# mit-acl/roman

Hardware: AMD Instinct MI355X
Metric: submap-pair alignments/sec + p50 latency at n=m=200 objects, d=512 (higher is better)
Workload: dtype f64 (fixed-point SpMV sums); 1 GPU; config 3: batch of 256 submap pairs per GPU, n=200 m=200 d=512, method=semanticgrav (xyz + 512-d descriptors + gravity prior); p50 latency measured on config 2 (single pair); pairs_per_call=256, n=200, m=200, d=512, method=semanticgrav, batches_in_flight=3

## Files before the change

roman_amd/csrc/kernels.hip.h:

```cpp
#pragma once
#include <hip/hip_cooperative_groups.h>
#include <hip/hip_runtime.h>
#include <stdint.h>
#include <type_traits>
#include "../../include/roman_hip.h"

namespace roman {

constexpr int WAVE = 64;
constexpr int STREAM_MAXL = 3072;

struct DevParams {
    roman_params_t p;
    double sig2;
    double sin_unc;
    double x_eps;
    double x_mindist;
    int32_t single;
    int32_t gravity;
    int32_t F;
    int32_t max_compact;
    int32_t gmode;
    int32_t diag_one;
    int32_t keep_all;
// ... 2625 lines not shown
            }
            queued += (uint32_t)__popcll(act);
            while (queued >= 64u * FILL_E) evaluate(64u * FILL_E);
        }
    }
    while (queued > 0u) evaluate(min(queued, 64u * (uint32_t)FILL_E));
    return upper;
}

template <bool GRAV, typename IdxT, bool QUAD>
__global__ void __launch_bounds__(1024) k_fill(DevParams D, const ProbDesc* __restrict__ probs,
                                               ProbState* __restrict__ st,
                                               const BatchTotals* __restrict__ tot,
                                               const ItemDesc* __restrict__ items,
                                               const double* __restrict__ tabPool,
                                               const int32_t* __restrict__ li, const int32_t* __restrict__ lj,
                                               const double* __restrict__ ls,
                                               const double* __restrict__ lza, const double* __restrict__ lzb,
                                               const uint32_t* __restrict__ rowCnt,
                                               const unsigned long long* __restrict__ maskPool,
                                               const uint32_t* __restrict__ prefPool,
                                               const uint32_t* __restrict__ rowPos,
                                               const uint32_t* __restrict__ sliceWidth,
                                               const uint32_t* __restrict__ sliceBase,
                                               IdxT* __restrict__ cols, double* __restrict__ vals, int TC, int RPB ,
                                               const uint32_t* __restrict__ permPool )
{
    extern __shared__ __attribute__((aligned(16))) unsigned char smem[];
    double* cS = reinterpret_cast<double*>(smem);
    double* cZa = cS + TC;
    double* cZb = cZa + (GRAV ? TC : 0);
    int32_t* cI = reinterpret_cast<int32_t*>(cZb + (GRAV ? TC : 0));
    int32_t* cJ = cI + TC;
    uint32_t* cBase = reinterpret_cast<uint32_t*>(cJ + TC);
    uint32_t* cPos = cBase + TC;
    uint32_t* rings = cPos + TC;
    const int tid = threadIdx.x, nt = blockDim.x;
    const int lane = tid & 63, w = tid >> 6, wpb = nt >> 6;
    FillRows R;
    R.s = reinterpret_cast<double*>(rings + (size_t)wpb * 3 * FILL_Q); R.za = R.s + FILL_RPB; R.zb = R.za + FILL_RPB;
    R.k = reinterpret_cast<int32_t*>(R.zb + FILL_RPB); R.i = R.k + FILL_RPB; R.j = R.i + FILL_RPB; R.base = reinterpret_cast<uint32_t*>(R.j + FILL_RPB);
    uint32_t* qK = rings + (size_t)w * 3 * FILL_Q;
    uint32_t* qQ = qK + FILL_Q;
    uint32_t* qE = qQ + FILL_Q;
    const int nItems = tot->items;
    const int gpu_ = max(1, FILL_RPB / RPB);
    const int nUnits = (nItems + gpu_ - 1) / gpu_;
    const int Gx_ = (nUnits + 7) >> 3;
    for (int sIdx_ = blockIdx.x; (sIdx_ >> 3) < Gx_; sIdx_ += gridDim.x) {
        const int u_ = (sIdx_ & 7) * Gx_ + (sIdx_ >> 3);
        if (u_ >= nUnits) continue;
        const int tEnd_ = min(nItems, (u_ + 1) * gpu_);
        for (int t = u_ * gpu_; t < tEnd_; ) {
        ItemDesc it = items[t];
        const int b = it.b;
        int te_ = t + 1;
        while (te_ < tEnd_ && items[te_].b == b) ++te_;
        const int nIt_ = te_ - t;
        t = te_;
        if (uni_i(st[b].kind) == 1) {
        const ProbDesc pd = probs[b];
        const int L = st[b].L;
        const int64_t lo = pd.liveOff, mo = st[b].maskOff, no = st[b].nnzOff;
        const int nrows = min(nIt_ * RPB, L - it.row0);
        const double* TA = tabPool + pd.tabOff;
        const double* TB = TA + (int64_t)pd.n1 * pd.n1;
        const bool ldscol = L <= TC;
        __syncthreads();
        for (int r = tid; r < nrows; r += nt) {
            const uint32_t pos = (uint32_t)(it.row0 + r);
            const int k = (int)permPool[lo + pos];
            R.k[r] = k; R.i[r] = li[lo + k]; R.j[r] = lj[lo + k]; R.s[r] = ls[lo + k];
            if (GRAV) { R.za[r] = lza[lo + k]; R.zb[r] = lzb[lo + k]; }
            R.base[r] = sliceBase[lo + (pos >> 6)] + (pos & 63u);
        }
        if (ldscol) {
            for (int q = tid; q < L; q += nt) {
                cI[q] = li[lo + q]; cJ[q] = lj[lo + q]; cS[q] = ls[lo + q];
                if (GRAV) { cZa[q] = lza[lo + q]; cZb[q] = lzb[lo + q]; }
                const uint32_t pos = rowPos[lo + q];
                cBase[q] = sliceBase[lo + (pos >> 6)] + (pos & 63u); cPos[q] = pos;
            }
        }
        __syncthreads();
        uint32_t upper = 0u;
        if (ldscol)
            upper = fill_item<GRAV, IdxT, 1, QUAD>(D, pd, L, it.row0, nrows, 0, (L + 63) >> 6, w, wpb, lane, cI, cJ, cS, cZa, cZb, cBase, cPos, TA, TB,
                                                maskPool + mo, prefPool + mo, R, qK, qQ, qE, cols + no, vals + no);
        else {
            const int TCw = TC & ~63;
            for (int q0 = 0; q0 < L; q0 += TCw) {
                const int qn = min(TCw, L - q0);
                if (q0 > 0) __syncthreads();
                for (int q = tid; q < qn; q += nt) {
                    const int64_t g_ = lo + q0 + q;
                    cI[q] = li[g_]; cJ[q] = lj[g_]; cS[q] = ls[g_];
                    if (GRAV) { cZa[q] = lza[g_]; cZb[q] = lzb[g_]; }
                    cPos[q] = rowPos[g_];
                }
                __syncthreads();
                upper += fill_item<GRAV, IdxT, 2, QUAD>(D, pd, L, it.row0, nrows, q0, (qn + 63) >> 6, w, wpb, lane, cI, cJ, cS, cZa, cZb, cBase, cPos, TA, TB,
                                                        maskPool + mo, prefPool + mo, R, qK, qQ, qE, cols + no, vals + no);
            }
        }
        for (int r = w; r < nrows; r += wpb) {
            const uint32_t pos = (uint32_t)(it.row0 + r);
            const int k = (int)permPool[lo + pos];
            const uint32_t width = sliceWidth[lo + (pos >> 6)];
            const int64_t sb = no + sliceBase[lo + (pos >> 6)];
            for (uint32_t e = rowCnt[lo + k] + lane; e < width; e += WAVE) {
                cols[col_pos<QUAD>(sb, pos & 63u, e)] = fb_inert<IdxT>(pos);
                vals[val_pos<QUAD>(sb, pos & 63u, e)] = 0.0;
            }
        }
        if (QUAD && it.row0 + nrows == L && (L & 63)) {
            const uint32_t sl = (uint32_t)(L >> 6);
            const uint32_t width = sliceWidth[lo + sl];
            const int64_t sb = no + sliceBase[lo + sl];
            const uint32_t nfree = 64u - (uint32_t)(L & 63);
            for (uint32_t x = tid; x < nfree * width; x += nt) {
                const uint32_t slot = (uint32_t)(L & 63) + x / width, e = x % width;
                cols[col_pos<QUAD>(sb, slot, e)] = fb_inert<IdxT>(0u);
                vals[val_pos<QUAD>(sb, slot, e)] = 0.0;
            }
        }
        for (int off = 32; off > 0; off >>= 1) upper += __shfl_xor(upper, off);
        if (lane == 0 && upper) atomicAdd(&st[b].nnzUpper, (unsigned long long)upper);
        }
        }
    }
}

constexpr int FILLS_MAXSPI = STREAM_MAXL / 64;

template <bool GRAV, bool FAST>
__device__ __forceinline__ double fill_value(const DevParams& D, double a, double bb, double dza, double dzb, double ss, double sk, double sq)
{
    double c;
    if (GRAV && D.gmode != 3) {
        const double ch = fabs(a - bb);
        const double hm = a > bb ? a : bb;
        double cv = fabs(dza - dzb) - D.sin_unc * hm;
        if (cv < 0.0) cv = 0.0;
        c = sqrt(ch * ch + cv * cv);
    } else {
        c = fabs(a - bb);
    }
    const double sa = fx_exp(((-0.5 * c) * c) / D.sig2);
    if (FAST) return (sa == 0.0) ? 0.0 : fx_cbrt(sa * ss);
    return fuse_pair(D, sa, sk, sq);
}

constexpr uint32_t FILL_ROTATE = 5;

template <bool GRAV, bool FAST, bool OBJ>
__global__ void __launch_bounds__(1024) k_fill_list(DevParams D, int B, const ProbDesc* __restrict__ probs,
                                                    ProbState* __restrict__ st, const BatchTotals* __restrict__ tot,
                                                    const double* __restrict__ tabPool, const double* __restrict__ feats, int NO ,
                                                    const int32_t* __restrict__ li, const int32_t* __restrict__ lj,
                                                    const double* __restrict__ ls,
                                                    const double* __restrict__ lza, const double* __restrict__ lzb,
                                                    const uint16_t* __restrict__ listPool, const uint32_t* __restrict__ listOff,
                                                    const uint32_t* __restrict__ rowCnt,
                                                    const uint32_t* __restrict__ perm, const uint32_t* __restrict__ rowPos,
                                                    const uint32_t* __restrict__ sliceWidth,
                                                    const uint32_t* __restrict__ sliceBase,
                                                    uint16_t* __restrict__ cols, double* __restrict__ vals, int TC, int NG, int SPI )
{
    extern __shared__ __attribute__((aligned(16))) unsigned char smem[];
    double* cS = reinterpret_cast<double*>(smem);
    dbl2_t* sO = reinterpret_cast<dbl2_t*>(cS + TC);
    double* cZa = OBJ ? cS + TC + 8 * NO : cS + TC;
    double* cZb = cZa + ((GRAV && !OBJ) ? TC : 0);
    int32_t* cI = reinterpret_cast<int32_t*>(cZb + ((GRAV && !OBJ) ? TC : 0));
    int32_t* cJ = cI + TC;
    uint32_t* gK = reinterpret_cast<uint32_t*>(cJ + TC);
    uint32_t* gCnt = gK + SPI * 64;
    uint32_t* gOff = gCnt + SPI * 64;
    uint32_t* gQ = gOff + SPI * 64;
    uint32_t* gSB = gQ + SPI + 1;
    uint16_t* cP = reinterpret_cast<uint16_t*>(gSB + SPI + 1);
    const int tid = threadIdx.x, nt = blockDim.x;
    const int lane = tid & 63, w = tid >> 6, nw = nt >> 6;
    const int nGroups = tot->sliceGroups;
    const int Gx = (nGroups + 7) >> 3;
    for (int sIdx = blockIdx.x; (sIdx >> 3) < Gx; sIdx += gridDim.x) {
        const int t = (sIdx & 7) * Gx + (sIdx >> 3);
        if (t < nGroups) {
        int b = 0;
        {
            int lo_ = 0, hi_ = B - 1;
            while (lo_ < hi_) { const int mid = (lo_ + hi_ + 1) >> 1; if (st[mid].sgBase <= t) lo_ = mid; else hi_ = mid - 1; }
            b = lo_;
        }
        const ProbDesc pd = probs[b];
        const int L = st[b].L;
        const int W = (L + 63) >> 6;
        const int64_t lo = pd.liveOff, no = st[b].nnzOff;
        const uint16_t* lists = listPool + st[b].listOff;
        const int ngb = min(NG, W), spib = (W + ngb - 1) / max(ngb, 1);
        const int s_begin = (t - st[b].sgBase) * spib, s_end = min(W, s_begin + spib), ns = max(s_end - s_begin, 0);
        const double* TA = tabPool + pd.tabOff;
        const double* TB = TA + (int64_t)pd.n1 * pd.n1;
        __syncthreads();
        for (int q = tid; q < L; q += nt) {
            cI[q] = li[lo + q]; cJ[q] = lj[lo + q]; cS[q] = ls[lo + q]; cP[q] = (uint16_t)rowPos[lo + q];
            if (GRAV && !OBJ) { cZa[q] = lza[lo + q]; cZb[q] = lzb[lo + q]; }
        }
        if (OBJ) {
            const int pdim = D.p.point_dim;
            for (int o = tid; o < pd.n1 + pd.n2; o += nt) {
                const double* f = feats + (o < pd.n1 ? pd.off1 + o : pd.off2 + (o - pd.n1)) * D.F;
                const int slot = o < pd.n1 ? o : NO + (o - pd.n1);
                sO[2 * slot] = dbl2_t{f[0], pdim > 1 ? f[1] : 0.0};
                sO[2 * slot + 1] = dbl2_t{pdim > 2 ? f[2] : 0.0, 0.0};
            }
        }
        const bool horiz = D.gmode == 1 || D.gmode == 2;
        for (int x = tid; x < ns * 64; x += nt) {
            const int p = s_begin * 64 + x;
            const bool row = p < L;
            gK[x] = row ? perm[lo + p] : 0xffffffffu; gCnt[x] = row ? rowCnt[lo + p] : 0u; gOff[x] = row ? listOff[lo + p] : 0u;
        }
        if (w == 0) {
            const uint32_t wq = (lane < ns) ? (sliceWidth[lo + s_begin + lane] >> 2) : 0u;
            const uint32_t ex = wave_excl_scan(wq, lane);
            if (lane < ns) { gQ[lane] = ex; gSB[lane] = sliceBase[lo + s_begin + lane]; }
            if (lane == ns) gQ[ns] = ex;
        }
        __syncthreads();
        const uint32_t Q = gQ[ns];
        uint32_t upper = 0;
        int si = 0;
        for (uint32_t u = (uint32_t)w; u < Q; u += (uint32_t)nw) {
            while (u >= gQ[si + 1]) ++si;
            const uint32_t g = u - gQ[si];
            const int64_t sb = no + gSB[si];
            const int x = si * 64 + lane;
            const uint32_t kraw = gK[x], cnt = gCnt[x];
            const uint32_t nq = (cnt + 3u) >> 2;
            uint32_t e0 = g << 2;
            if (g < nq) e0 = ((g + (uint32_t)x * FILL_ROTATE) % nq) << 2;
            uint2 qq = make_uint2(0u, 0u);
            if (e0 < cnt) qq = *reinterpret_cast<const uint2*>(lists + gOff[x] + e0);
            const int k = (kraw == 0xffffffffu) ? 0 : (int)kraw;
            const double sk = cS[k];
            const double* TAr = TA + (int64_t)cI[k] * pd.n1;
            const double* TBr = TB + (int64_t)cJ[k] * pd.n2;
            const double zak = (GRAV && !OBJ) ? cZa[k] : 0.0, zbk = (GRAV && !OBJ) ? cZb[k] : 0.0;
            dbl2_t oa0 = {0.0, 0.0}, oa1 = {0.0, 0.0}, ob0 = {0.0, 0.0}, ob1 = {0.0, 0.0};
            if (OBJ) { oa0 = sO[2 * cI[k]]; oa1 = sO[2 * cI[k] + 1]; ob0 = sO[2 * (NO + cJ[k])]; ob1 = sO[2 * (NO + cJ[k]) + 1]; }
            const uint32_t inert = ((uint32_t)L + (uint32_t)lane) | 0x8000u;
            uint32_t cw[4]; double vv[4];
#pragma unroll
            for (int j = 0; j < 4; ++j) {
                const bool have = e0 + (uint32_t)j < cnt;
                const uint32_t qr = ((j < 2 ? qq.x : qq.y) >> (16 * (j & 1))) & 0xffffu;
                const int q = have ? (int)qr : k;
                double a, bb, dza, dzb;
                if (OBJ) {
                    const dbl2_t pa0 = sO[2 * cI[q]], pa1 = sO[2 * cI[q] + 1], pb0 = sO[2 * (NO + cJ[q])], pb1 = sO[2 * (NO + cJ[q]) + 1];
                    const double dxa = oa0.x - pa0.x, dya = oa0.y - pa0.y, dxb = ob0.x - pb0.x, dyb = ob0.y - pb0.y;
                    dza = oa1.x - pa1.x; dzb = ob1.x - pb1.x;
                    const double h2a = dxa * dxa + dya * dya, h2b = dxb * dxb + dyb * dyb;
                    a = horiz ? sqrt(h2a) : sqrt(h2a + dza * dza);
                    bb = horiz ? sqrt(h2b) : sqrt(h2b + dzb * dzb);
                } else {
                    a = TAr[cI[q]]; bb = TBr[cJ[q]];
                    dza = GRAV ? zak - cZa[q] : 0.0; dzb = GRAV ? zbk - cZb[q] : 0.0;
                }
                if (!have) { a = 0.0; bb = 0.0; }
                const double sq = cS[q];
                const double v = fill_value<GRAV, FAST>(D, a, bb, GRAV ? dza : 0.0, GRAV ? dzb : 0.0, sk * sq, sk, sq);
                const bool keep = have && v > D.p.affinityeps;
                cw[j] = keep ? (uint32_t)cP[q] : inert;
                vv[j] = keep ? v : 0.0;
                upper += keep ? 1u : 0u;
            }
            *reinterpret_cast<uint2*>(cols + sb + (int64_t)g * 256 + lane * 4) = make_uint2(cw[0] | (cw[1] << 16), cw[2] | (cw[3] << 16));
            *reinterpret_cast<double2*>(vals + sb + (int64_t)(2 * g) * 128 + lane * 2) = make_double2(vv[0], vv[1]);
            *reinterpret_cast<double2*>(vals + sb + (int64_t)(2 * g + 1) * 128 + lane * 2) = make_double2(vv[2], vv[3]);
        }
        for (int off = 32; off > 0; off >>= 1) upper += __shfl_xor(upper, off);
        if (lane == 0 && upper) atomicAdd(&st[b].nnzUpper, (unsigned long long)upper);
        }
    }
}

__device__ __forceinline__ void dense_entry(const double* __restrict__ M, const double* __restrict__ C, int n, int k, int q, double& mv, double& cv)
{
    const int a = min(k, q), b = max(k, q);
    mv = M[(int64_t)a * n + b]; cv = C[(int64_t)a * n + b];
}

__global__ void __launch_bounds__(256) k_dense_mask(int n, const double* __restrict__ M, const double* __restrict__ C,
                                                    unsigned long long* __restrict__ mask ,
                                                    int* __restrict__ flags )
{
    const int lane = threadIdx.x & 63;
    const int W = (n + 63) >> 6;
    const int nwaves = (int)(gridDim.x * (blockDim.x >> 6));
    for (int k = (int)(blockIdx.x * (blockDim.x >> 6) + (threadIdx.x >> 6)); k < n; k += nwaves) {
        bool cz = false;
        for (int w = 0; w < W; ++w) {
            const int q = (w << 6) + lane;
            bool cand = false;
            if (q < n && q != k) {
                double mv, cv;
                dense_entry(M, C, n, k, q, mv, cv);
                cand = (mv != 0.0) || (cv != 0.0);
                cz = cz || (cand && cv == 0.0);
            }
            const unsigned long long m = __ballot(cand);
            if (lane == 0) mask[(int64_t)k * W + w] = m;
        }
        if (__ballot(cz) != 0ull && lane == 0) atomicOr(flags, 1);
    }
}

__global__ void __launch_bounds__(256) k_dense_range(int n, const double* __restrict__ M, int* __restrict__ flags)
{
    const int lane = threadIdx.x & 63;
    const int nwaves = (int)(gridDim.x * (blockDim.x >> 6));
    bool bad = false;
    for (int k = (int)(blockIdx.x * (blockDim.x >> 6) + (threadIdx.x >> 6)); k < n; k += nwaves)
        for (int q = k + 1 + lane; q < n; q += 64) {
            const double v = M[(int64_t)k * n + q];
            bad = bad || !(v >= 0.0 && v <= 1.0);
        }
    if (__ballot(bad) != 0ull && lane == 0) atomicOr(flags + 1, 1);
}

template <int KIND>
__global__ void __launch_bounds__(256) k_dense_fill(int n, const double* __restrict__ M, const double* __restrict__ C,
                                                    ProbState* __restrict__ st,
                                                    const uint32_t* __restrict__ rowCnt, const uint32_t* __restrict__ rowPos, const uint32_t* __restrict__ perm,
                                                    const uint32_t* __restrict__ sliceWidth, const uint32_t* __restrict__ sliceBase,
                                                    const uint16_t* __restrict__ listPool, const uint32_t* __restrict__ listOff,
                                                    const unsigned long long* __restrict__ mask, const uint32_t* __restrict__ pref,
                                                    uint16_t* __restrict__ cols16, uint32_t* __restrict__ cols32, double* __restrict__ vals)
{
    const uint32_t total = st[0].nnzCap;
    const int64_t no = st[0].nnzOff;
    const int nsl = (n + 63) >> 6, W = nsl;
    const uint16_t* lists = listPool + st[0].listOff;
    unsigned upper = 0;
    for (uint32_t t = blockIdx.x * blockDim.x + threadIdx.x; t < total; t += gridDim.x * blockDim.x) {
        int sl = 0;
        {
            int lo_ = 0, hi_ = nsl - 1;
            while (lo_ < hi_) { const int mid = (lo_ + hi_ + 1) >> 1; if (sliceBase[mid] <= t) lo_ = mid; else hi_ = mid - 1; }
            sl = lo_;
        }
        const uint32_t sb = sliceBase[sl], off = t - sb;
        const uint32_t slot = (off & 255u) >> 2, e = ((off >> 8) << 2) | (off & 3u);
        const int pos = sl * 64 + (int)slot;
        const int k = pos < n ? (int)perm[pos] : -1;
        double val = 0.0;
        if (KIND == 0) {
            uint32_t label = ((uint32_t)n + slot) | 0x8000u;
            if (k >= 0 && e < rowCnt[pos]) {
                const int q = (int)lists[listOff[pos] + e];
                double mv, cv;
                dense_entry(M, C, n, k, q, mv, cv);
                label = rowPos[q] | (cv == 0.0 ? 0x8000u : 0u); val = mv; ++upper;
            }
            cols16[no + t] = (uint16_t)label;
        } else {
            uint32_t label = (uint32_t)(k >= 0 ? pos : 0) | 0x80000000u;
            if (k >= 0 && e < rowCnt[k]) {
                const unsigned long long* mrow = mask + (int64_t)k * W;
                const uint32_t* prow = pref + (int64_t)k * W;
                int lo_ = 0, hi_ = W - 1;
                while (lo_ < hi_) { const int mid = (lo_ + hi_ + 1) >> 1; if (prow[mid] <= e) lo_ = mid; else hi_ = mid - 1; }
                unsigned long long m = mrow[lo_];
                for (uint32_t i = prow[lo_]; i < e; ++i) m &= m - 1ull;
                const int q = (lo_ << 6) + __builtin_ctzll(m);
                double mv, cv;
                dense_entry(M, C, n, k, q, mv, cv);
                label = rowPos[q] | (cv == 0.0 ? 0x80000000u : 0u); val = mv;
                if (q > k) ++upper;
            }
            cols32[no + t] = label;
        }
        vals[no + val_pos<true>(sb, slot, e)] = val;
    }
    for (int off = 32; off > 0; off >>= 1) upper += __shfl_xor(upper, off);
    if ((threadIdx.x & 63) == 0 && upper) atomicAdd(&st[0].nnzUpper, (unsigned long long)upper);
}


struct SolveOut {
    int32_t* assoc_out; int32_t* n_assoc_out; double* T_out; int32_t* status_out;
    roman_stats_t* stats_out; int32_t kmax;
    int32_t* nodesOrig;
    int32_t* nSel;
    double*  uOut;
    unsigned long long* dbg;
};

__device__ __forceinline__ void block_sum2(double& a, double& b, double* red, int& par, int tid, int nw)
{
    for (int off = 32; off > 0; off >>= 1) { a += __shfl_xor(a, off); b += __shfl_xor(b, off); }
    double* rr = red + 32 * par;
    par ^= 1;
    if ((tid & 63) == 0) { rr[2 * (tid >> 6)] = a; rr[2 * (tid >> 6) + 1] = b; }
    __syncthreads();
    double ra = 0.0, rb = 0.0;
    for (int i = 0; i < nw; ++i) { ra += rr[2 * i]; rb += rr[2 * i + 1]; }
    a = ra; b = rb;
}

typedef unsigned int uint4_t __attribute__((ext_vector_type(4)));
template <typename IdxT, int G>
__device__ __forceinline__ void spmv_sell(const double* u, int L, const uint32_t* __restrict__ perm,
                                          const uint32_t* __restrict__ sliceWidth, const uint32_t* __restrict__ sliceBase,
                                          const IdxT* __restrict__ cols, const double* __restrict__ vals,
                                          double* Mu, double* Cu, int tid, int nt)
{
    static_assert(sizeof(IdxT) == 4, "fallback layout: 32-bit column words");
    const int lane = tid & 63, w = tid >> 6, nw = nt >> 6;
    const int nsl = (L + 63) >> 6;
    for (int s = w; s < nsl; s += nw) {
        const int pos = (s << 6) + lane;
        const bool valid = pos < L;
        const uint32_t nq = sliceWidth[s] >> 2;
        const uint4_t* cp = reinterpret_cast<const uint4_t*>(cols + sliceBase[s]) + lane;
        const dbl2_t* vp = reinterpret_cast<const dbl2_t*>(vals + sliceBase[s]) + lane;
        double am = 0.0, ac = 0.0;
        for (uint32_t g0 = 0; g0 < nq; g0 += G) {
            uint4_t c_[G]; dbl2_t v0_[G], v1_[G];
#pragma unroll
            for (int t = 0; t < G; ++t) {
                const uint32_t g = min(g0 + (uint32_t)t, nq - 1u);
// ... 3927 lines not shown
```

roman_amd/csrc/roman_hip.hip:

```cpp
#include <hip/hip_runtime.h>
#include <algorithm>
#include <cmath>
#include <cstdarg>
#include <cstdint>
#include <cstdio>
#include <cstdlib>
#include <cstring>
#include <new>
#include <string>
#include <vector>

#include "kernels.hip.h"

using namespace roman;

namespace {

thread_local std::string g_last_error;

struct DevBuf {
    void* p = nullptr; size_t cap = 0;
    hipError_t ensure(size_t bytes) {
        if (bytes <= cap) return hipSuccess;
        if (p) { hipError_t e = hipFree(p); p = nullptr; cap = 0; if (e != hipSuccess) return e; }
// ... 589 lines not shown
    const int Lneed = (expL + 255) & ~255;
    const int NRc = ((size_t)16 * 2 * ldsPerRow * sizeof(double) + (size_t)std::min(Lneed, 2048) * colBytesC <= c->lds_max) ? 2 : 1;
    int wpb = 16;
    while (wpb > 1 && (size_t)wpb * NRc * ldsPerRow * sizeof(double) + 256 * colBytesC > c->lds_max) wpb >>= 1;
    if ((size_t)wpb * NRc * ldsPerRow * sizeof(double) + 256 * colBytesC > c->lds_max)
        return fail(c, ROMAN_E_TOO_LARGE, "maps of %d objects exceed the LDS table staging of this build", maxN);
    const int ldsPerWave = NRc * ldsPerRow;
    const size_t tabLds = (size_t)wpb * ldsPerWave * sizeof(double);
    int TCc = (int)std::min<size_t>((c->lds_max - tabLds) / colBytesC, 32768) & ~255;
    TCc = std::min(TCc, Lneed);
    const size_t pairLds = tabLds + (size_t)TCc * colBytesC;
    const int pairGrid = c->num_cu * std::max(1, std::min(2048 / (wpb * 64), (int)(c->lds_max / pairLds)));
    int preNR = 0, preWpb = 0, preTC = 0; size_t preLds = 0;
    const int preRow = (2 * std::max(maxN, 1) + 1 + 3) & ~3;
    {
        const char* preEnv = getenv("ROMAN_COUNT_PRE");
        const bool want = (preEnv ? preEnv[0] != '0' : true) && D.pre_invw > 0.0 && std::isfinite(D.pre_invw) && Lneed <= (preEnv ? 16000 : 4096) && maxN <= 32767;
        if (want) {
            const int tc = Lneed;
            for (int wp = PRE_WAVES; wp >= 8; wp -= 4) {
                const size_t need = (size_t)(tc + PRE_COLPAD + 4) * 4 + (size_t)wp * (size_t)count_pre_wave_bytes(preRow, tc);
                if (need <= c->lds_max) { preNR = PRE_NR; preWpb = wp; preTC = tc; preLds = need; break; }
            }
        }
    }

    StageTimer t1(c, ROMAN_STAGE_COUNT_PASS);
    {
        static const char* fusedEnv = getenv("ROMAN_SMALL_FUSED");
        const bool want = smallOut != nullptr && !(fusedEnv && fusedEnv[0] == '0') && D.p.maxiniters >= 1 && D.p.maxlsiters >= 1 && maxTab > 0 &&
                          (c->hist.valid ? c->hist.smallSeen : maxA <= 16 * SMALL_MAXL);
        if (want) {
            SolveOut O;
            int rc = make_solve_out(c, B, sumA, *smallOut, &O);
            if (rc) return rc;
            HIPCHK(c, hipMemsetAsync(WS.queue.as<int>() + 8, 0, sizeof(int), WS.stream));
            const bool fast = D.single && (D.p.single_mode == ROMAN_SINGLE_BOTH || D.p.single_mode == ROMAN_SINGLE_OFFDIAG) && D.p.distance_weight == 1.0 &&
                              D.p.fusion_method != ROMAN_FUSE_ARITHMETIC_MEAN && D.p.fusion_method != ROMAN_FUSE_PRODUCT;
            constexpr size_t ldsSmall = small_lds_bytes();
            const int grid = std::max(1, std::min(B, c->num_cu * 12));
            auto ks = fast ? k_small<true> : k_small<false>;
            hipLaunchKernelGGL(ks, dim3(grid), dim3(64), ldsSmall, WS.stream, D, B, dP, dS, in.feats, in.assoc, WS.tabPool.as<double>(),
                               LP.lp, LP.li, LP.lj, LP.ls, LP.ld, LP.lza, LP.lzb, WS.plp.as<int32_t>(), WS.pld.as<double>(), WS.rowPos.as<uint32_t>(),
                               smallU0, O, WS.queue.as<int>() + 8);
    DBG(c, "k_small");
            static const char* onlyEnv = getenv("ROMAN_SMALL_ONLY");
            D.small_only = (c->hist.valid && !c->hist.generalSeen && !(onlyEnv && onlyEnv[0] == '0')) ? 1 : 0;
            Dout->small_only = D.small_only;
        }
    }
    hipLaunchKernelGGL(k_rowbase, dim3(1), dim3(B > 256 ? 1024 : 256), 0, WS.stream, B, RPB, SZ.capMaskWords, dS, dT, D.small_only, cosScreen ? (const int32_t*)WS.cosDense.as<int32_t>() : (const int32_t*)nullptr);
    DBG(c, "k_rowbase");
    if (!D.small_only) {
    hipLaunchKernelGGL(k_items, dim3(B), dim3(256), 0, WS.stream, RPB, dS, WS.items.as<ItemDesc>());
    DBG(c, "k_items");
    }
    if (sumA > 0 && !D.small_only) {
        const bool needTiled = D.allow_fallback || TCc < Lneed;
        int degGiven = 0;
        for (int tiled = 0; tiled < (needTiled ? 2 : 1); ++tiled) {
            const void* kc = nullptr;
#define ROMAN_KC(GM_) kc = tiled ? (NRc == 2 ? reinterpret_cast<const void*>(k_count<GM_, 2, true>) : reinterpret_cast<const void*>(k_count<GM_, 1, true>)) \
                                 : (NRc == 2 ? reinterpret_cast<const void*>(k_count<GM_, 2, false>) : reinterpret_cast<const void*>(k_count<GM_, 1, false>))
            switch (D.gmode) { case 1: ROMAN_KC(1); break; case 2: ROMAN_KC(2); break; case 3: ROMAN_KC(3); break; default: ROMAN_KC(0); break; }
#undef ROMAN_KC
            const bool usePre = !tiled && preNR > 0;
            if (usePre) {
#define ROMAN_KP(GM_) kc = reinterpret_cast<const void*>(k_count<GM_, 1, false, true>)
                switch (D.gmode) { case 1: ROMAN_KP(1); break; case 2: ROMAN_KP(2); break; case 3: ROMAN_KP(3); break; default: ROMAN_KP(0); break; }
#undef ROMAN_KP
            }
            const size_t ldsK = usePre ? preLds : pairLds;
            const int wpbK = usePre ? preWpb : wpb;
            const int gridK = usePre ? c->num_cu * std::max(1, std::min(2048 / (wpbK * 64), (int)(c->lds_max / ldsK))) : pairGrid;
            const char* wholeEnv = getenv("ROMAN_COUNT_WHOLE");
            const bool wholeP = usePre && (wholeEnv ? wholeEnv[0] != '0' : B >= c->num_cu) && preLds + (size_t)preTC * 4 <= c->lds_max;
            if (wholeP) degGiven = 1;
            HIPCHK(c, dyn_lds(c, kc, ldsK + (wholeP ? (size_t)preTC * 4 : 0)));
            DevParams a_D = D; const ProbDesc* a_dP = dP; const ProbState* a_dS = dS; const BatchTotals* a_dT = dT; const ItemDesc* a_items = WS.items.as<ItemDesc>();
            const double* a_tab = WS.tabPool.as<double>(); const int32_t* a_li = LP.li; const int32_t* a_lj = LP.lj; const double* a_za = LP.lza; const double* a_zb = LP.lzb;
            uint32_t* a_rc = WS.rowCnt.as<uint32_t>(); unsigned long long* a_mask = WS.maskPool.as<unsigned long long>(); uint32_t* a_pref = WS.prefPool.as<uint32_t>();
            int a_TC = usePre ? preTC : TCc, a_lpw = usePre ? preRow : ldsPerWave;
            int a_RPB = wholeP ? -B : RPB;
            const uint16_t* a_qtab = WS.qtabPool.as<uint16_t>();
            void* args[] = {&a_D, &a_dP, &a_dS, &a_dT, &a_items, &a_tab, &a_li, &a_lj, &a_za, &a_zb, &a_rc, &a_mask, &a_pref, &a_TC, &a_lpw, &a_RPB, &a_qtab};
            HIPCHK(c, hipLaunchKernel(kc, dim3(gridK), dim3(wpbK * 64), args, ldsK + (wholeP ? (size_t)preTC * 4 : 0), WS.stream));
        }
    DBG(c, "k_count");
        const char* listsEnv = getenv("ROMAN_LISTS");
        const int fusedLists = listsEnv ? (listsEnv[0] == '0' ? 0 : 1) : (B >= std::max(8, c->num_cu / 8) ? 1 : 0);
        if (fusedLists) {
            static size_t listsStatic = 0;
            if (listsStatic == 0) {
                hipFuncAttributes fa;
                HIPCHK(c, hipFuncGetAttributes(&fa, reinterpret_cast<const void*>(k_lists)));
                listsStatic = std::max<size_t>(fa.sharedSizeBytes, 1);
            }
            const char* llEnv = getenv("ROMAN_LISTS_LDS");
            const size_t room = c->lds_max > listsStatic ? c->lds_max - listsStatic : 0;
            const size_t winBytes = std::min(room, llEnv ? (size_t)std::max(0, atoi(llEnv)) : room) & ~(size_t)15;
            if (winBytes) HIPCHK(c, dyn_lds(c, reinterpret_cast<const void*>(k_lists), winBytes));
            hipLaunchKernelGGL(k_lists, dim3((unsigned)std::max(1, std::min(B, 2 * c->num_cu))), dim3(LISTS_NT), winBytes, WS.stream, B, dP, dS, dT,
                               WS.maskPool.as<unsigned long long>(), WS.listPool.as<uint16_t>(), WS.listOff.as<uint32_t>(),
                               WS.rowCnt.as<uint32_t>(), WS.perm.as<uint32_t>(), WS.rowPos.as<uint32_t>(), LP, PP, (long long)SZ.capList, sort_eq_max(), degGiven,
                               (int)(winBytes / sizeof(uint16_t)));
    DBG(c, "k_lists");
        }
        if (!fusedLists || D.allow_fallback) {
        {
            const int Wexp = (expL + 63) / 64;
            const int tasks = ((Wexp + 7) / 8) * ((std::max(Wexp - 1, 1) + 7) / 8);
            const int T = std::max(tasks, 1);
            hipLaunchKernelGGL(k_mirror, dim3((unsigned)(T * ((B + 7) / 8) * 8)), dim3(512), 0, WS.stream, B, T, dS, WS.maskPool.as<unsigned long long>(), fusedLists);
    DBG(c, "k_mirror");
        }
        hipLaunchKernelGGL(k_rowprefix, dim3(c->num_cu * 2), dim3(1024), 0, WS.stream, dP, dS, dT, WS.items.as<ItemDesc>(),
                           WS.maskPool.as<unsigned long long>(), WS.prefPool.as<uint32_t>(), WS.rowCnt.as<uint32_t>(), RPB, fusedLists);
    DBG(c, "k_rowprefix");
        int sortThr = 1024;
        if (!D.allow_fallback) { int N2 = 64; while (N2 < expL) N2 <<= 1; sortThr = std::max(64, std::min(1024, N2 / 2)); }
        hipLaunchKernelGGL(k_rowsort, dim3(B), dim3(sortThr), 0, WS.stream, dP, dS, dT, WS.rowCnt.as<uint32_t>(), WS.rowPos.as<uint32_t>(), WS.perm.as<uint32_t>(),
                           WS.sliceWidth.as<uint32_t>(), WS.sliceBase.as<uint32_t>(), WS.listOff.as<uint32_t>(), SZ.capList, fusedLists, sort_eq_max());
    DBG(c, "k_rowsort");
        if (!fusedLists) {
        const int upThr = expL <= 256 ? 256 : 1024;
        hipLaunchKernelGGL(k_upper, dim3(c->num_cu * 2 * (1024 / upThr)), dim3(upThr), 0, WS.stream, dP, dS, dT, WS.items.as<ItemDesc>(),
                           WS.maskPool.as<unsigned long long>(), WS.listPool.as<uint16_t>(), WS.listOff.as<uint32_t>(),
                           WS.rowCnt.as<uint32_t>(), WS.perm.as<uint32_t>(), WS.rowPos.as<uint32_t>(), LP, PP, RPB);
    DBG(c, "k_upper");
        }
        }
        hipLaunchKernelGGL(k_slicegeom, dim3(B), dim3(64), 0, WS.stream, dP, dS, WS.rowCnt.as<uint32_t>(), WS.sliceWidth.as<uint32_t>(), WS.sliceBase.as<uint32_t>());
    DBG(c, "k_slicegeom");
    }
    int NG = (int)std::max<int64_t>(1, std::min<int64_t>(FILLS_MAXSPI, (3 * (int64_t)c->num_cu + B / 2) / std::max(B, 1)));
    {
        const int stride = std::max(1, (c->num_cu & ~7) / 8);
        auto gcd = [](int a, int b) { while (b) { const int t = a % b; a = b; b = t; } return a; };
        while (NG > 1 && gcd(stride % NG, NG) != 1) --NG;
    }
    const int Wmax = std::max(1, D.stream_maxL / 64);
    const int SPI = (Wmax + std::min(NG, Wmax) - 1) / std::min(NG, Wmax);
    if (!D.small_only) {
    hipLaunchKernelGGL(k_probscan, dim3(1), dim3(B > 256 ? 1024 : 256), 0, WS.stream, B, NG, SZ.capNnz, dS, dT);
    DBG(c, "k_probscan");
    }
    t1.stop();

    StageTimer t2(c, ROMAN_STAGE_FILL);
    if (sumA > 0 && !D.small_only) {
        const int colBytesF = D.gravity ? 32 : 16;
        const int TCs = D.stream_maxL;
        const int NO = (std::max(maxN, 1) + 1) & ~1;
        const size_t groupLds = sizeof(uint32_t) * (size_t)(3 * SPI * 64 + 2 * (SPI + 1) + 2);
        const bool obj = (size_t)TCs * (16 + 2) + (size_t)64 * NO + groupLds <= c->lds_max;
        const size_t sliceLds = obj ? (size_t)TCs * (16 + 2) + (size_t)64 * NO + groupLds : (size_t)TCs * (colBytesF + 2) + groupLds;
        if (sliceLds > c->lds_max) return fail(c, ROMAN_E_TOO_LARGE, "internal: stream column tile does not fit the LDS");
        const bool fast = D.single && (D.p.single_mode == ROMAN_SINGLE_BOTH || D.p.single_mode == ROMAN_SINGLE_OFFDIAG) && D.p.distance_weight == 1.0 &&
                          D.p.fusion_method != ROMAN_FUSE_ARITHMETIC_MEAN && D.p.fusion_method != ROMAN_FUSE_PRODUCT;
        auto kf = D.gravity ? (fast ? k_fill_list<true, true, false> : k_fill_list<true, false, false>) : (fast ? k_fill_list<false, true, false> : k_fill_list<false, false, false>);
        if (obj) kf = D.gravity ? (fast ? k_fill_list<true, true, true> : k_fill_list<true, false, true>) : (fast ? k_fill_list<false, true, true> : k_fill_list<false, false, true>);
        HIPCHK(c, dyn_lds(c, reinterpret_cast<const void*>(kf), sliceLds));
        const int fillThr = expL <= 256 ? 256 : 1024;
        const int fillWgs = std::max(1, std::min(1024 / fillThr, (int)(c->lds_max / sliceLds)));
        hipLaunchKernelGGL(kf, dim3((unsigned)((c->num_cu & ~7) * fillWgs)), dim3(fillThr), sliceLds, WS.stream,
                           D, B, dP, dS, dT, WS.tabPool.as<double>(), in.feats, NO, LP.li, LP.lj, LP.ls, LP.lza, LP.lzb,
                           WS.listPool.as<uint16_t>(), WS.listOff.as<uint32_t>(), WS.rowCnt.as<uint32_t>(), WS.perm.as<uint32_t>(), WS.rowPos.as<uint32_t>(),
                           WS.sliceWidth.as<uint32_t>(), WS.sliceBase.as<uint32_t>(), WS.cols16.as<uint16_t>(), WS.vals.as<double>(), TCs, NG, SPI);
    DBG(c, "k_fill_list");
        if (D.allow_fallback && (SZ.maxA > D.stream_maxL || D.p.maxiniters < 1 || D.p.maxlsiters < 1)) {
            const int colBytesG = D.gravity ? 40 : 24;
            const size_t ringLds = (size_t)16 * 3 * FILL_Q * sizeof(uint32_t) + (size_t)FILL_RPB * FILL_ROWBYTES;
            static_assert(FILL_RPB >= 128, "the work items of a batch are blocks of at most 128 rows");
            int TCf = (int)std::min<size_t>((c->lds_max - ringLds) / colBytesG, 32768) & ~63;
            TCf = std::min(TCf, std::max(64, (Lneed + 63) & ~63));
            const size_t fillLds = ringLds + (size_t)TCf * colBytesG;
            const int fillGrid = c->num_cu * std::max(1, std::min(2, (int)(c->lds_max / fillLds)));
            if (D.idx16) {
                auto kg = D.gravity ? k_fill<true, uint16_t, true> : k_fill<false, uint16_t, true>;
                HIPCHK(c, dyn_lds(c, reinterpret_cast<const void*>(kg), fillLds));
                hipLaunchKernelGGL(kg, dim3(fillGrid), dim3(1024), fillLds, WS.stream, D, dP, dS, dT, WS.items.as<ItemDesc>(), WS.tabPool.as<double>(),
                                   LP.li, LP.lj, LP.ls, LP.lza, LP.lzb,
                                   WS.rowCnt.as<uint32_t>(), WS.maskPool.as<unsigned long long>(), WS.prefPool.as<uint32_t>(), WS.rowPos.as<uint32_t>(),
                                   WS.sliceWidth.as<uint32_t>(), WS.sliceBase.as<uint32_t>(), WS.cols16.as<uint16_t>(), WS.vals.as<double>(), TCf, RPB, (const uint32_t*)WS.perm.as<uint32_t>());
            } else {
                auto kg = D.gravity ? k_fill<true, uint32_t, true> : k_fill<false, uint32_t, true>;
                HIPCHK(c, dyn_lds(c, reinterpret_cast<const void*>(kg), fillLds));
                hipLaunchKernelGGL(kg, dim3(fillGrid), dim3(1024), fillLds, WS.stream, D, dP, dS, dT, WS.items.as<ItemDesc>(), WS.tabPool.as<double>(),
                                   LP.li, LP.lj, LP.ls, LP.lza, LP.lzb,
                                   WS.rowCnt.as<uint32_t>(), WS.maskPool.as<unsigned long long>(), WS.prefPool.as<uint32_t>(), WS.rowPos.as<uint32_t>(),
                                   WS.sliceWidth.as<uint32_t>(), WS.sliceBase.as<uint32_t>(), WS.cols32.as<uint32_t>(), WS.vals.as<double>(), TCf, RPB, (const uint32_t*)WS.perm.as<uint32_t>());
            }
    DBG(c, "k_fill");
        }
    }
    t2.stop();
    HIPCHK(c, hipMemcpyAsync(WS.pinnedTotals, dT, sizeof(BatchTotals), hipMemcpyDeviceToHost, WS.stream));
    HIPCHK(c, hipEventRecord(WS.totEvent, WS.stream));
    WS.totPending = true; WS.totMaskBound = SZ.maskBound; WS.totSumA = SZ.sumA; WS.totMaxA = SZ.maxA; WS.totEpoch = c->histEpoch;
    HIPCHK(c, hipGetLastError());
    return ROMAN_OK;
}

int enqueue_solve(roman_ctx* c, const DevParams& D, int B, int64_t sumA, int64_t maxA , const double* feats, const int32_t* assoc,
                  const double* u0, bool hascz, int mayFallback , const BatchOut& out)
{
    const size_t R1 = (size_t)std::max<int64_t>(sumA, 1);
    SolveOut O;
    { int rc_ = make_solve_out(c, B, sumA, out, &O); if (rc_) return rc_; }
#ifdef ROMAN_SOLVE_TIMING
    HIPCHK(c, WS.hAux3.ensure(sizeof(unsigned long long) * 16 * (size_t)B));
    HIPCHK(c, hipMemsetAsync(WS.hAux3.p, 0, sizeof(unsigned long long) * 16 * (size_t)B, WS.stream));
    O.dbg = WS.hAux3.as<unsigned long long>();
#endif
    constexpr int NW = SOLVE_WAVES;
    const int Lc = STREAM_MAXL + 64;
    const size_t ldsUp = (size_t)3 * 8 * Lc + sizeof(double) * red_doubles(NW) + sizeof(uint32_t) * (ST_MAXSL + 2) + sizeof(int) * 8 + 16;
    const int wgPerCu = std::max(1, std::min((int)(c->lds_max / ldsUp), 2048 / (NW * 64)));
    const int gridUp = std::max(1, std::min(B, c->num_cu * wgPerCu));

    StageTimer t3(c, ROMAN_STAGE_SOLVE);
    const bool coopPlanned = mayFallback && D.wide != 0 && c->coop_ok;
    if (coopPlanned) {
        HIPCHK(c, WS.wideBar.ensure(sizeof(unsigned) * WIDE_BAR_WORDS));
        HIPCHK(c, WS.fbList.ensure(sizeof(int32_t) * (size_t)B));
        HIPCHK(c, hipMemsetAsync(WS.wideBar.p, 0, sizeof(unsigned) * WIDE_BAR_WORDS, WS.stream));
    }
    hipLaunchKernelGGL(k_skipped, dim3((unsigned)((B + 255) / 256)), dim3(256), 0, WS.stream, B, WS.probs.as<ProbDesc>(), WS.state.as<ProbState>(), O, WS.queue.as<int>(),
                       coopPlanned ? WS.fbList.as<int32_t>() : (int32_t*)nullptr, coopPlanned ? WS.wideBar.as<unsigned>() : (unsigned*)nullptr);
    DBG(c, "k_skipped");
    if (D.small_only) { t3.stop(); HIPCHK(c, hipGetLastError()); return ROMAN_OK; }
    static const char* smallEnv = getenv("ROMAN_SMALL");
    const bool small = !(smallEnv && smallEnv[0] == '0') && D.p.maxiniters >= 1 && D.p.maxlsiters >= 1 &&
                       (c->hist.valid ? c->hist.smallSeen : maxA <= 16 * SMALL_MAXL);
    const int Lc1 = SMALL_MAXL + 64;
    const size_t ldsUp1 = (size_t)3 * 8 * Lc1 + sizeof(double) * red_doubles(1) + sizeof(uint32_t) * (ST_MAXSL + 2) + sizeof(int) * 8 + 16 + (size_t)COO_CAP * 12;
    const int gridUp1 = std::max(1, std::min(B, c->num_cu * 24));
#define ROMAN_LAUNCH_UP(CZ_)                                                                                                  \
    do {                                                                                                                      \
        auto kup = k_solve_up<NW, CZ_, STREAM_MAXL>;                                                                          \
        HIPCHK(c, dyn_lds(c, reinterpret_cast<const void*>(kup), ldsUp)); \
        hipLaunchKernelGGL(kup, dim3(gridUp), dim3(NW * 64), ldsUp, WS.stream, D, B, WS.probs.as<ProbDesc>(), WS.state.as<ProbState>(), feats, assoc, \
                           WS.plp.as<int32_t>(), WS.lp.as<int32_t>(), WS.rowPos.as<uint32_t>(), WS.pld.as<double>(), WS.sliceBase.as<uint32_t>(), \
                           WS.cols16.as<uint16_t>(), WS.vals.as<double>(), u0, O, WS.queue.as<int>(), Lc, small ? SMALL_MAXL + 1 : 0, STREAM_MAXL, (small && c->hist.valid && !c->hist.largeSeen) ? 64 : 1); \
        if (small) {                                                                                                          \
            HIPCHK(c, dyn_lds(c, reinterpret_cast<const void*>(k_solve_up<1, CZ_, SMALL_MAXL>), ldsUp1));                       \
            hipLaunchKernelGGL((k_solve_up<1, CZ_, SMALL_MAXL>), dim3(gridUp1), dim3(64), ldsUp1, WS.stream, D, B, WS.probs.as<ProbDesc>(), WS.state.as<ProbState>(), feats, assoc, \
                               WS.plp.as<int32_t>(), WS.lp.as<int32_t>(), WS.rowPos.as<uint32_t>(), WS.pld.as<double>(), WS.sliceBase.as<uint32_t>(), \
                               WS.cols16.as<uint16_t>(), WS.vals.as<double>(), u0, O, WS.queue.as<int>() + 1, Lc1, 0, SMALL_MAXL, 1); \
        }                                                                                                                     \
    } while (0)
    if (hascz) ROMAN_LAUNCH_UP(true); else ROMAN_LAUNCH_UP(false);
#undef ROMAN_LAUNCH_UP
    DBG(c, "k_solve_up");
    if (mayFallback) {
        HIPCHK(c, WS.vMu.ensure(sizeof(double) * R1)); HIPCHK(c, WS.vCu.ensure(sizeof(double) * R1));
        HIPCHK(c, WS.vMun.ensure(sizeof(double) * R1)); HIPCHK(c, WS.vCun.ensure(sizeof(double) * R1));
        HIPCHK(c, WS.gU.ensure(sizeof(double) * R1)); HIPCHK(c, WS.gUn.ensure(sizeof(double) * R1));
        bool coop = D.wide != 0 && c->coop_ok;
        if (coop) {
            const int G = c->num_cu;
            int a_teams = 0;
            const int perXcd = std::max(1, (G + c->num_xcc - 1) / c->num_xcc);
            {
                constexpr int margin = 2;
                auto cap = [&](int sub) { return (int64_t)WIDE_KW * std::max(1, perXcd / sub - margin) * WIDE_NW * 64; };
                if (mayFallback >= 2 && maxA <= cap(1)) {
                    a_teams = 1;
                    for (int s_ = 2; s_ <= 4; ++s_) if (mayFallback > 6 * s_ && maxA <= cap(s_)) a_teams = s_;
                    if (a_teams == 2 && mayFallback > 18 && G == c->num_cu && maxA <= (int64_t)WIDE_KW * (perXcd / 3) * WIDE_NW * 64) a_teams = 3;
                }
                const char* teamEnv = getenv("ROMAN_WIDE_TEAMS");
                const int forced = teamEnv ? atoi(teamEnv) : c->wide_teams;
                if (teamEnv || c->wide_teams >= 0) a_teams = (forced >= 1 && forced <= 4 && mayFallback >= 1 && maxA <= cap(forced)) ? forced : 0;
            }
            if (a_teams) c->teams_launched = true;
            const int nTeams = a_teams ? 8 * a_teams : 1;
            const int NWGt = a_teams ? std::min(G, 2 * ((perXcd + a_teams - 1) / a_teams) + 8) * WIDE_NW : G * WIDE_NW;
            int a_ucfg = (D.idx16 && a_teams > 0 && maxA >= 8000) ? 1 : 0;
            { const char* e_ = getenv("ROMAN_WIDE_UPPER"); if (e_ && e_[0]) a_ucfg = (D.idx16 && e_[0] != '0') ? 1 : 0; }
            long long a_partStride = (long long)(((size_t)NWGt * WIDE_MAXCH + (size_t)(a_ucfg ? WIDE_MAXBLK : 1) * ((size_t)(maxA + 63) / 64) + 4) * 64 * 2);
            HIPCHK(c, WS.widePart.ensure(sizeof(double) * (size_t)a_partStride * (size_t)nTeams));
            HIPCHK(c, WS.wideSlots.ensure(sizeof(double) * 2 * (size_t)G * WIDE_NRED * (size_t)nTeams));
            DevParams Dv = D; int Bv = B;
            const ProbDesc* a_probs = WS.probs.as<ProbDesc>(); ProbState* a_state = WS.state.as<ProbState>();
            const double* a_feats = feats; const int32_t* a_assoc = assoc;
            const int32_t* a_lp = WS.lp.as<int32_t>(); const double* a_ld = WS.ld.as<double>();
            const uint32_t* a_perm = WS.perm.as<uint32_t>(); const uint32_t* a_rpos = WS.rowPos.as<uint32_t>(); const uint32_t* a_sb = WS.sliceBase.as<uint32_t>();
            const void* a_cols = D.idx16 ? (const void*)WS.cols16.as<uint16_t>() : (const void*)WS.cols32.as<uint32_t>(); const double* a_vals = WS.vals.as<double>();
            double* a_vU = WS.gU.as<double>(); double* a_vX = WS.gUn.as<double>(); double* a_vX2 = WS.vCun.as<double>();
            double* a_s0 = WS.vMu.as<double>(); double* a_s1 = WS.vCu.as<double>(); double* a_s2 = WS.vMun.as<double>();
            int32_t* a_plp = WS.plp.as<int32_t>();
            const double* a_u0 = u0; SolveOut a_O = O;
            double* a_part = WS.widePart.as<double>(); double* a_slots = WS.wideSlots.as<double>(); unsigned* a_bar = WS.wideBar.as<unsigned>();
            int a_bmw = (int)((maxA + 63) / 64) + 1;
            HIPCHK(c, WS.wideBm.ensure(sizeof(unsigned long long) * 3 * (size_t)a_bmw * (size_t)nTeams));
            unsigned long long* a_bm = WS.wideBm.as<unsigned long long>();
            const int64_t wideFixed = (int64_t)wide_fixed_lds(a_bmw);
            int a_xcap = (int)(((int64_t)c->lds_max - 4096 - wideFixed) / (int64_t)sizeof(double)) & ~63;
            if (a_xcap < 0) a_xcap = 0;
            const size_t wideLds = sizeof(double) * (size_t)a_xcap + (size_t)wideFixed;
            int a_ccfg = 6 | (128 << 8) | (4 << 16);
            { const char* e_ = getenv("ROMAN_WIDE_COMPACT"); if (e_ && e_[0]) a_ccfg = (int)strtol(e_, nullptr, 0); }
            int a_ySlots = NWGt / WIDE_NW;
            int a_ycap = a_ucfg ? ((a_xcap / 3) & ~63) : 0;
            if (a_ucfg && a_ycap < 64) a_ucfg = 0;
            if (a_ucfg) {
// ... 2670 lines not shown
```

Before: 180,200 alignments/s.

## Compact live fill work across slices so waves process only non-padding list quads

The sliced fill kernel used to give each wave one quad-group of a 64-row slice, so lanes whose row had no list entries at that depth sat idle or wrote padding. It now processes windows of 256 quad-groups: a ballot marks live lanes, padding entries are written directly, a prefix scan over live counts builds a compacted index, and every lane then takes one live (row, group) pair found by binary search and nth-set-bit. This is meant to cut lane divergence and wasted ALU work on skewed row lengths. The cost is extra barriers per window, more LDS, scattered rather than coalesced stores, and search overhead.

```diff
diff --git a/roman_amd/csrc/kernels.hip.h b/roman_amd/csrc/kernels.hip.h
--- a/roman_amd/csrc/kernels.hip.h
+++ b/roman_amd/csrc/kernels.hip.h
@@ -2801,6 +2801,20 @@
 }
 
 constexpr uint32_t FILL_ROTATE = 5;
+constexpr int FILL_WIN = 256;
+
+__device__ __forceinline__ uint32_t nth_set_bit(uint32_t lo, uint32_t hi, uint32_t n)
+{
+    uint32_t base = 0, v = lo;
+    const uint32_t c = (uint32_t)__popc(lo);
+    if (n >= c) { n -= c; v = hi; base = 32; }
+#pragma unroll
+    for (int s = 16; s > 0; s >>= 1) {
+        const uint32_t cl = (uint32_t)__popc(v & ((1u << s) - 1u));
+        if (n >= cl) { n -= cl; v >>= s; base += (uint32_t)s; }
+    }
+    return base;
+}
 
 template <bool GRAV, bool FAST, bool OBJ>
 __global__ void __launch_bounds__(1024) k_fill_list(DevParams D, int B, const ProbDesc* __restrict__ probs,
@@ -2828,7 +2842,11 @@
     uint32_t* gOff = gCnt + SPI * 64;
     uint32_t* gQ = gOff + SPI * 64;
     uint32_t* gSB = gQ + SPI + 1;
-    uint16_t* cP = reinterpret_cast<uint16_t*>(gSB + SPI + 1);
+    uint32_t* wLo = gSB + SPI + 1;
+    uint32_t* wHi = wLo + FILL_WIN;
+    uint32_t* wSl = wHi + FILL_WIN;
+    uint32_t* wPre = wSl + FILL_WIN;
+    uint16_t* cP = reinterpret_cast<uint16_t*>(wPre + FILL_WIN + 1);
     const int tid = threadIdx.x, nt = blockDim.x;
     const int lane = tid & 63, w = tid >> 6, nw = nt >> 6;
     const int nGroups = tot->sliceGroups;
@@ -2880,26 +2898,62 @@
         __syncthreads();
         const uint32_t Q = gQ[ns];
         uint32_t upper = 0;
-        int si = 0;
-        for (uint32_t u = (uint32_t)w; u < Q; u += (uint32_t)nw) {
-            while (u >= gQ[si + 1]) ++si;
-            const uint32_t g = u - gQ[si];
+        int si1 = 0;
+        for (uint32_t u0 = 0; u0 < Q; u0 += (uint32_t)FILL_WIN) {
+            const uint32_t Wn = min((uint32_t)FILL_WIN, Q - u0);
+            if (u0) __syncthreads();
+            for (uint32_t ul = (uint32_t)w; ul < Wn; ul += (uint32_t)nw) {
+                const uint32_t u = u0 + ul;
+                while (u >= gQ[si1 + 1]) ++si1;
+                const uint32_t g = u - gQ[si1];
+                const bool live = g < ((gCnt[si1 * 64 + lane] + 3u) >> 2);
+                const unsigned long long m = __ballot(live);
+                if (lane == 0) { wLo[ul] = (uint32_t)m; wHi[ul] = (uint32_t)(m >> 32); wSl[ul] = (uint32_t)si1; wPre[ul] = (uint32_t)__popcll(m); }
+                if (!live) {
+                    const int64_t sb = no + gSB[si1];
+                    const uint32_t inert = ((uint32_t)L + (uint32_t)lane) | 0x8000u, i2 = inert | (inert << 16);
+                    *reinterpret_cast<uint2*>(cols + sb + (int64_t)g * 256 + lane * 4) = make_uint2(i2, i2);
+                    *reinterpret_cast<double2*>(vals + sb + (int64_t)(2 * g) * 128 + lane * 2) = make_double2(0.0, 0.0);
+                    *reinterpret_cast<double2*>(vals + sb + (int64_t)(2 * g + 1) * 128 + lane * 2) = make_double2(0.0, 0.0);
+                }
+            }
+            for (uint32_t ul = Wn + (uint32_t)tid; ul < (uint32_t)FILL_WIN; ul += (uint32_t)nt) wPre[ul] = 0u;
+            __syncthreads();
+            if (w == 0) {
+                static_assert(FILL_WIN == 4 * WAVE, "one wave scans the window, four slot quads per lane");
+                uint32_t c[4], s = 0;
+#pragma unroll
+                for (int j = 0; j < 4; ++j) { c[j] = wPre[4 * lane + j]; s += c[j]; }
+                uint32_t ex = wave_excl_scan(s, lane);
+#pragma unroll
+                for (int j = 0; j < 4; ++j) { wPre[4 * lane + j] = ex; ex += c[j]; }
+                if (lane == WAVE - 1) wPre[FILL_WIN] = ex;
+            }
+            __syncthreads();
+            const uint32_t F = wPre[FILL_WIN];
+            for (uint32_t f0 = (uint32_t)uni_i(w) * 64u; f0 < F; f0 += (uint32_t)nt) {
+            uint32_t ul = 0;
+            { uint32_t lo_ = 0, hi_ = Wn - 1u; while (lo_ < hi_) { const uint32_t mid = (lo_ + hi_ + 1u) >> 1; if (wPre[mid] <= f0) lo_ = mid; else hi_ = mid - 1u; } ul = lo_; }
+            const uint32_t f = f0 + (uint32_t)lane;
+            if (f < F) {
+            while (wPre[ul + 1] <= f) ++ul;
+            const int r = (int)nth_set_bit(wLo[ul], wHi[ul], f - wPre[ul]);
+            const int si = (int)wSl[ul];
+            const uint32_t g = u0 + ul - gQ[si];
             const int64_t sb = no + gSB[si];
-            const int x = si * 64 + lane;
+            const int x = si * 64 + r;
             const uint32_t kraw = gK[x], cnt = gCnt[x];
             const uint32_t nq = (cnt + 3u) >> 2;
-            uint32_t e0 = g << 2;
-            if (g < nq) e0 = ((g + (uint32_t)x * FILL_ROTATE) % nq) << 2;
-            uint2 qq = make_uint2(0u, 0u);
-            if (e0 < cnt) qq = *reinterpret_cast<const uint2*>(lists + gOff[x] + e0);
-            const int k = (kraw == 0xffffffffu) ? 0 : (int)kraw;
+            const uint32_t e0 = ((g + (uint32_t)x * FILL_ROTATE) % nq) << 2;
+            const uint2 qq = *reinterpret_cast<const uint2*>(lists + gOff[x] + e0);
+            const int k = (int)kraw;
             const double sk = cS[k];
             const double* TAr = TA + (int64_t)cI[k] * pd.n1;
             const double* TBr = TB + (int64_t)cJ[k] * pd.n2;
             const double zak = (GRAV && !OBJ) ? cZa[k] : 0.0, zbk = (GRAV && !OBJ) ? cZb[k] : 0.0;
             dbl2_t oa0 = {0.0, 0.0}, oa1 = {0.0, 0.0}, ob0 = {0.0, 0.0}, ob1 = {0.0, 0.0};
             if (OBJ) { oa0 = sO[2 * cI[k]]; oa1 = sO[2 * cI[k] + 1]; ob0 = sO[2 * (NO + cJ[k])]; ob1 = sO[2 * (NO + cJ[k]) + 1]; }
-            const uint32_t inert = ((uint32_t)L + (uint32_t)lane) | 0x8000u;
+            const uint32_t inert = ((uint32_t)L + (uint32_t)r) | 0x8000u;
             uint32_t cw[4]; double vv[4];
 #pragma unroll
             for (int j = 0; j < 4; ++j) {
@@ -2926,9 +2980,11 @@
                 vv[j] = keep ? v : 0.0;
                 upper += keep ? 1u : 0u;
             }
-            *reinterpret_cast<uint2*>(cols + sb + (int64_t)g * 256 + lane * 4) = make_uint2(cw[0] | (cw[1] << 16), cw[2] | (cw[3] << 16));
-            *reinterpret_cast<double2*>(vals + sb + (int64_t)(2 * g) * 128 + lane * 2) = make_double2(vv[0], vv[1]);
-            *reinterpret_cast<double2*>(vals + sb + (int64_t)(2 * g + 1) * 128 + lane * 2) = make_double2(vv[2], vv[3]);
+            *reinterpret_cast<uint2*>(cols + sb + (int64_t)g * 256 + r * 4) = make_uint2(cw[0] | (cw[1] << 16), cw[2] | (cw[3] << 16));
+            *reinterpret_cast<double2*>(vals + sb + (int64_t)(2 * g) * 128 + r * 2) = make_double2(vv[0], vv[1]);
+            *reinterpret_cast<double2*>(vals + sb + (int64_t)(2 * g + 1) * 128 + r * 2) = make_double2(vv[2], vv[3]);
+            }
+            }
         }
         for (int off = 32; off > 0; off >>= 1) upper += __shfl_xor(upper, off);
         if (lane == 0 && upper) atomicAdd(&st[b].nnzUpper, (unsigned long long)upper);
diff --git a/roman_amd/csrc/roman_hip.hip b/roman_amd/csrc/roman_hip.hip
--- a/roman_amd/csrc/roman_hip.hip
+++ b/roman_amd/csrc/roman_hip.hip
@@ -765,7 +765,7 @@
         const int colBytesF = D.gravity ? 32 : 16;
         const int TCs = D.stream_maxL;
         const int NO = (std::max(maxN, 1) + 1) & ~1;
-        const size_t groupLds = sizeof(uint32_t) * (size_t)(3 * SPI * 64 + 2 * (SPI + 1) + 2);
+        const size_t groupLds = sizeof(uint32_t) * (size_t)(3 * SPI * 64 + 2 * (SPI + 1) + 4 * FILL_WIN + 1 + 2);
         const bool obj = (size_t)TCs * (16 + 2) + (size_t)64 * NO + groupLds <= c->lds_max;
         const size_t sliceLds = obj ? (size_t)TCs * (16 + 2) + (size_t)64 * NO + groupLds : (size_t)TCs * (colBytesF + 2) + groupLds;
         if (sliceLds > c->lds_max) return fail(c, ROMAN_E_TOO_LARGE, "internal: stream column tile does not fit the LDS");
```

Result: faster. 182,600 alignments/s (median of 6 runs) (+1.3%).
